# schlawg/fishnet

Measured on AMD Instinct MI355X. Metric: NNUE positions evaluated/sec (1–8 MI355X) + % HBM roofline, bit-exact, higher is better.
Workload: dtype int16

## Files before the change

### fishnet_amd/csrc/ft_sliced.hip

```cpp
#include <hip/hip_runtime.h>

#include <type_traits>

#include "sliced_common.h"

namespace fnnue {

namespace {

__global__ __launch_bounds__(1024) void plan_count_kernel(const fnnue_pos* __restrict__ pos, uint32_t n,
                                                         uint32_t* __restrict__ ctr, uint32_t* __restrict__ err) {
  __shared__ uint32_t h[kBins];
  for (int i = threadIdx.x; i < kBins; i += blockDim.x) h[i] = 0;
  __syncthreads();
  uint32_t bad = 0;
  for (uint32_t p = blockIdx.x * blockDim.x + threadIdx.x; p < n; p += gridDim.x * blockDim.x) {
    const LaneBoard b = lane_decode<false>(pos + p);
    if (!b.ok) {
      bad = 1;
      atomicAdd(&h[kItemBins + 8], 1u);
    } else {
      atomicAdd(&h[king_block(0, b.wk) * 33 + b.cnt], 1u);
      atomicAdd(&h[king_block(1, b.bk) * 33 + b.cnt], 1u);
      atomicAdd(&h[kItemBins + ((b.cnt - 1) >> 2)], 1u);
    }
  }
  if (__ballot(bad) && (threadIdx.x & 63) == 0) atomicOr(err, 1u);
  __syncthreads();
  for (int i = threadIdx.x; i < kBins; i += blockDim.x)
    if (h[i]) atomicAdd(&ctr[kCnt + i], h[i]);
}

__global__ __launch_bounds__(kScatterPositions) void plan_scatter_kernel(const fnnue_pos* __restrict__ pos, uint32_t n,
                                                           uint32_t* __restrict__ ctr, uint32_t* __restrict__ items,
                                                           uint16_t* __restrict__ flist, uint32_t* __restrict__ perm,
                                                           uint8_t* __restrict__ bucket_out,
                                                           int32_t* __restrict__ psqt_out) {
  __shared__ uint32_t lcnt[kBins];
  __shared__ uint32_t lbase[kBins];
  __shared__ uint32_t lists[kScatterPositions * kListStrideWords];
  for (int i = threadIdx.x; i < kBins; i += blockDim.x) lcnt[i] = 0;
  __syncthreads();
  const uint32_t p = blockIdx.x * kScatterPositions + threadIdx.x;
  const bool live = p < n;
  LaneBoard b;
  int kw = 0, kb = 0, kp = kItemBins + 8;
  uint32_t rw = 0, rb = 0, rp = 0;
  if (live) {
    b = lane_decode(pos + p);
    if (b.ok) {
      kw = king_block(0, b.wk) * 33 + b.cnt;
      kb = king_block(1, b.bk) * 33 + b.cnt;
      kp = kItemBins + ((b.cnt - 1) >> 2);
      rw = atomicAdd(&lcnt[kw], 1u);
      rb = atomicAdd(&lcnt[kb], 1u);
    }
    rp = atomicAdd(&lcnt[kp], 1u);
  }
  __syncthreads();
  for (int i = threadIdx.x; i < kBins; i += blockDim.x)
    lbase[i] = lcnt[i] ? atomicAdd(&ctr[kCur + i], lcnt[i]) : 0;
  __syncthreads();
  if (!live) return;
  const uint32_t slot = lbase[kp] + rp;
  perm[slot] = p;
  if (!b.ok) {
    bucket_out[slot] = 0xFF;
    psqt_out[p] = 0;
    return;
  }
  const int bucket = (b.cnt - 1) >> 2;
  const uint32_t iw = lbase[kw] + rw, ib = lbase[kb] + rb;
  uint32_t* mine = lists + threadIdx.x * kListStrideWords;
  write_rows(b, 0, b.wk, iw, (iw - ctr[kOff + king_block(0, b.wk) * 33]) & 1u, mine, flist);
  write_rows(b, 1, b.bk, ib, (ib - ctr[kOff + king_block(1, b.bk) * 33]) & 1u, mine, flist);
  items[iw] = ((uint32_t)b.cnt << 24) | ((uint32_t)bucket << 21) | (slot << 1) | (uint32_t)(b.stm != 0);
  items[ib] = ((uint32_t)b.cnt << 24) | ((uint32_t)bucket << 21) | (slot << 1) | (uint32_t)(b.stm != 1);
  bucket_out[slot] = (uint8_t)bucket;
}

template <int HD, bool kSwar, bool kPsqt, int kPStride, bool kClaim>
__device__ __forceinline__ uint32_t slice_pass(const PassFetch& f, uint2* __restrict__ lb, int lane, int it_in_wave,
                                               int s, int q, const char* base, u16x4 b_lo, u16x4 b_hi, int krow,
                                               const int32_t* ptile, __amdgpu_buffer_rsrc_t psqt_rsrc,
                                               __amdgpu_buffer_rsrc_t x_rsrc, uint32_t* next_pass) {
  constexpr int kLastItemLane = 48;
  const uint32_t rec = f.rec;
  const int maxn = (int)(__builtin_amdgcn_readlane(rec, kLastItemLane) >> 24);
  uint32_t claim = 0;
  if constexpr (kClaim) claim = claim_passes(next_pass, lane);
  lb[lane] = f.lst;
  uint32_t e[16];
  const uint4* my = reinterpret_cast<const uint4*>(lb) + 4 * it_in_wave;
#pragma unroll
  for (int m = 0; m < 4; ++m) {
    const uint4 v = my[m];
    e[4 * m] = v.x;
    e[4 * m + 1] = v.y;
    e[4 * m + 2] = v.z;
    e[4 * m + 3] = v.w;
  }
  u16x4 lo = b_lo, hi = b_hi;
  rows_sum<kSwar>(maxn - 1, e, base, lo, hi);
  const uint32_t xoff = (rec & kItemRowMask) * (HD / 2) + 32 * s + 4 * q;
  const uint32_t xv = kSwar ? transform4_swar(lo, hi) : transform4(lo, hi);
  __builtin_amdgcn_raw_buffer_store_b32(xv, x_rsrc, xoff, 0, 0);
  if constexpr (kPsqt) {
    const uint32_t li = (uint32_t)lane >> 3;
    const int src = (int)(((li & 4u) << 3) + ((0x10041400u >> (8u * (li & 3u))) & 0xFFu));
    const uint32_t reci = (uint32_t)__builtin_amdgcn_ds_bpermute(src << 2, (int)rec);
    const int bk = (int)((reci >> 21) & 7u);
    auto pw = [&](uint32_t en) { return (uint32_t)ptile[psqt_tile_word((int)(en >> 4), bk, kPStride)]; };
    uint32_t a2 = (lane & 7) == 0 ? (uint32_t)ptile[psqt_tile_word(krow, bk, kPStride)] : 0u;
    a2 += pw(f.lst.x & 0xFFFFu) + pw(f.lst.x >> 16) + pw(f.lst.y & 0xFFFFu) + pw(f.lst.y >> 16);
    a2 += (uint32_t)__builtin_amdgcn_mov_dpp((int)a2, 0xB1, 0xF, 0xF, false);
    a2 += (uint32_t)__builtin_amdgcn_mov_dpp((int)a2, 0x4E, 0xF, 0xF, false);
    a2 += (uint32_t)__builtin_amdgcn_mov_dpp((int)a2, 0x141, 0xF, 0xF, false);
    __builtin_amdgcn_raw_buffer_store_b32((int32_t)a2, psqt_rsrc,
                                          (lane & 7) == 0 ? (reci & kItemRowMask) * 4u : kDroppedOffset, 0, 0);
  }
  return claim;
}

#define FT_SLICES_LDS(G)                                                                                      \
  __shared__ uint4 img[G::kTileU4];                                                                           \
  __shared__ int32_t ptile[psqt_tile_words(G::kTileRows)];         \
  __shared__ uint2 lbuf[16][64];                                 \
  __shared__ uint32_t next_pass;

template <int HD, bool kSwar, class G>
__device__ __forceinline__ void ft_slices_body(uint4* img, int32_t* ptile, uint2 (*lbuf)[64], uint32_t* next_pass,
                                               const uint4* __restrict__ tiles,
                                               const int16_t* __restrict__ ftb, const uint32_t* __restrict__ ctr,
                                               const int4* __restrict__ units, const uint32_t* __restrict__ items,
                                               const uint16_t* __restrict__ flist, const int32_t* __restrict__ psqw,
                                               int32_t* __restrict__ psqt_part, uint8_t* __restrict__ x) {
  constexpr int S = HD / 64;
  constexpr int kTileU4 = G::kTileU4;
  const uint32_t w = blockIdx.x;
  const uint32_t j = w >> 3;
  const uint32_t unit = (j / S) * 8 + (w & 7);
  const int s = (int)(j % S);
  if (unit >= ctr[G::kNUnitsWord]) return;
  const int4 u = units[unit];
  const int lane = threadIdx.x & 63;
  const int wv = __builtin_amdgcn_readfirstlane(threadIdx.x >> 6);
  int it_in_wave, q;
  lane_item(lane, it_in_wave, q);
  constexpr int kTileLoads = (kTileU4 + 1023) / 1024;
  constexpr int kPStride = psqt_tile_stride(G::kTileRows);
  constexpr int kPtileU4 = psqt_fill_chunks(G::kTileRows), kPtileRealU4 = G::kRows * kPsqtBuckets / 4;
  static_assert(kPtileU4 <= 2048, "PSQT tile loads: two per thread");
  static_assert(kPStride % 32 == 4, "bucket b's rows start on bank 4 b");
  const uint4* src = tiles + ((size_t)u.x * S + s) * kTileU4;
  uint4 t[kTileLoads];
#pragma unroll
  for (int k = 0; k < kTileLoads; ++k)
    t[k] = src[min((int)threadIdx.x + 1024 * k, kTileU4 - 1)];
  uint4 pt[2];
  const uint4* psrc = reinterpret_cast<const uint4*>(psqw + (size_t)u.x * G::kRows * kPsqtBuckets);
  if (s == 0) {
#pragma unroll
    for (int k = 0; k < 2; ++k) pt[k] = psrc[min((int)threadIdx.x + 1024 * k, kPtileRealU4 - 1)];
  }
  u16x4 b_lo = *reinterpret_cast<const u16x4*>(ftb + 32 * s + 4 * q);
  u16x4 b_hi = *reinterpret_cast<const u16x4*>(ftb + HD / 2 + 32 * s + 4 * q);
  const int krow = G::king_row(u.x);
  const char* lbase = reinterpret_cast<const char*>(img) + G::kPlaneBytes * q;
  uint2* lb = lbuf[wv];
  const __amdgpu_buffer_rsrc_t psqt_rsrc = __builtin_amdgcn_make_buffer_rsrc(psqt_part, 0, kBufferRange, kBufferFlags);
  const __amdgpu_buffer_rsrc_t x_rsrc = __builtin_amdgcn_make_buffer_rsrc(x, 0, kBufferAll, kBufferFlags);
  const __amdgpu_buffer_rsrc_t items_rsrc =
      __builtin_amdgcn_make_buffer_rsrc(const_cast<uint32_t*>(items), 0, kBufferAll, kBufferFlags);
  const __amdgpu_buffer_rsrc_t flist_rsrc =
      __builtin_amdgcn_make_buffer_rsrc(const_cast<uint16_t*>(flist), 0, kBufferAll, kBufferFlags);
  const int last = u.z - 1;
  int base_a = u.y + wv * 8, base_b = base_a + 128;
  PassFetch fa = fetch_pass(items_rsrc, flist_rsrc, base_a, last, lane, it_in_wave);
  PassFetch fb = fetch_pass(items_rsrc, flist_rsrc, base_b, last, lane, it_in_wave);
#pragma unroll
  for (int k = 0; k < kTileLoads; ++k)
    if ((int)threadIdx.x + 1024 * k < kTileU4) {
      uint4 v = t[k];
      if constexpr (kSwar) v = swar_tile_words(v);
      img[threadIdx.x + 1024 * k] = v;
    }
  if (s == 0) {
#pragma unroll
    for (int k = 0; k < 2; ++k) {
      const int i = (int)threadIdx.x + 1024 * k;
      if (i < kPtileU4) {
        const uint4 v = i < kPtileRealU4 ? pt[k] : make_uint4(0, 0, 0, 0);
        const int r = psqt_fill_row(i);
        ptile[psqt_tile_word(r, psqt_fill_bucket(i, 0), kPStride)] = (int32_t)v.x;
        ptile[psqt_tile_word(r, psqt_fill_bucket(i, 1), kPStride)] = (int32_t)v.y;
        ptile[psqt_tile_word(r, psqt_fill_bucket(i, 2), kPStride)] = (int32_t)v.z;
        ptile[psqt_tile_word(r, psqt_fill_bucket(i, 3), kPStride)] = (int32_t)v.w;
      }
    }
  }
  if (threadIdx.x == 0) *next_pass = claim_start();
  __syncthreads();
  uint32_t claim = claim_passes(next_pass, lane);
  {
    const u32x4 kv = *reinterpret_cast<const u32x4*>(lbase + 16 * krow);
    if constexpr (kSwar) {
      b_lo = swar_words(b_lo);
      b_hi = swar_words_hi(b_hi);
    }
    accum_row<kSwar>(kv, b_lo, b_hi);
    if constexpr (kSwar) {
      b_lo = __builtin_bit_cast(u16x4, __builtin_bit_cast(u32x2, b_lo) + kSwarOffset);
      b_hi = __builtin_bit_cast(u16x4, __builtin_bit_cast(u32x2, b_hi) + kSwarOffset);
    }
  }
  auto run = [&](auto psqt) {
    constexpr bool kPsqt = decltype(psqt)::value;
    constexpr bool kClaimB = kClaimPasses == 1;
    while (base_a < u.z) {
      const PassFetch cur = fa;
      const int na = u.y + 8 * claimed_pass(claim);
      fa = fetch_pass(items_rsrc, flist_rsrc, na, last, lane, it_in_wave);
      claim = slice_pass<HD, kSwar, kPsqt, kPStride, true>(cur, lb, lane, it_in_wave, s, q, lbase, b_lo, b_hi, krow, ptile,
                                                           psqt_rsrc, x_rsrc, next_pass);
      base_a = na;
      if (base_b >= u.z) break;
      const PassFetch cur2 = fb;
      const int nb = kClaimPasses == 1 ? u.y + 8 * claimed_pass(claim) : na + 8;
      fb = fetch_pass(items_rsrc, flist_rsrc, nb, last, lane, it_in_wave);
      const uint32_t c2 = slice_pass<HD, kSwar, kPsqt, kPStride, kClaimB>(cur2, lb, lane, it_in_wave, s, q, lbase, b_lo,
                                                                          b_hi, krow, ptile, psqt_rsrc, x_rsrc, next_pass);
      if constexpr (kClaimB) claim = c2;
      base_b = nb;
    }
  };
  if (s == 0)
    run(std::true_type{});
  else
    run(std::false_type{});
}

template <int HD, bool kSwar, class G = ChessGeom>
__global__ __launch_bounds__(1024) void ft_slices_kernel(const uint4* __restrict__ tiles,
                                                         const int16_t* __restrict__ ftb,
                                                         const uint32_t* __restrict__ ctr,
                                                         const int4* __restrict__ units,
                                                         const uint32_t* __restrict__ items,
                                                         const uint16_t* __restrict__ flist,
                                                         const int32_t* __restrict__ psqw,
                                                         int32_t* __restrict__ psqt_part,
                                                         uint8_t* __restrict__ x) {
  FT_SLICES_LDS(G)
  ft_slices_body<HD, kSwar, G>(img, ptile, lbuf, &next_pass, tiles, ftb, ctr, units, items, flist, psqw, psqt_part, x);
}

template <int HD, class G = ChessGeom>
__global__ __launch_bounds__(1024) void ft_slices_mixed_kernel(const uint4* __restrict__ tiles,
                                                               const int16_t* __restrict__ ftb,
                                                               const uint32_t* __restrict__ ctr,
                                                               const int4* __restrict__ units,
                                                               const uint32_t* __restrict__ items,
                                                               const uint16_t* __restrict__ flist,
                                                               const int32_t* __restrict__ psqw,
                                                               int32_t* __restrict__ psqt_part,
                                                               uint8_t* __restrict__ x, uint64_t swar) {
  constexpr int S = HD / 64;
  FT_SLICES_LDS(G)
  const uint32_t s = (blockIdx.x >> 3) % S;
  if ((swar >> s) & 1)
    ft_slices_body<HD, true, G>(img, ptile, lbuf, &next_pass, tiles, ftb, ctr, units, items, flist, psqw, psqt_part, x);
  else
    ft_slices_body<HD, false, G>(img, ptile, lbuf, &next_pass, tiles, ftb, ctr, units, items, flist, psqw, psqt_part, x);
}

template <int HD>
hipError_t relayout_t(const NetPtrs& net, void* tiles, hipStream_t stream) {
  hipLaunchKernelGGL((relayout_kernel<HD>), dim3(2048), dim3(256), 0, stream, net.ft_w, (uint4*)tiles);
  return hipGetLastError();
}

template <int HD, class G = ChessGeom>
hipError_t ft_slices_t(const SlicedPlan& P, const NetPtrs& net, uint8_t* x, uint32_t max_units, hipStream_t stream) {
  constexpr int S = HD / 64;
  const uint32_t groups = (max_units + 7) / 8;
  const uint64_t all = (uint64_t(1) << S) - 1;
  if ((P.swar & all) == all)
    hipLaunchKernelGGL((ft_slices_kernel<HD, true, G>), dim3(groups * 8 * S), dim3(1024), 0, stream,
                       (const uint4*)P.tiles, net.ft_bias, P.ctr, (const int4*)P.units, P.items, P.flist, net.psqt_w,
                       P.psqt_part, x);
  else if ((P.swar & all) == 0)
    hipLaunchKernelGGL((ft_slices_kernel<HD, false, G>), dim3(groups * 8 * S), dim3(1024), 0, stream,
                       (const uint4*)P.tiles, net.ft_bias, P.ctr, (const int4*)P.units, P.items, P.flist, net.psqt_w,
                       P.psqt_part, x);
  else
    hipLaunchKernelGGL((ft_slices_mixed_kernel<HD, G>), dim3(groups * 8 * S), dim3(1024), 0, stream,
                       (const uint4*)P.tiles, net.ft_bias, P.ctr, (const int4*)P.units, P.items, P.flist, net.psqt_w,
                       P.psqt_part, x, P.swar);
  return hipGetLastError();
}

template <int HD, class G>
hipError_t relayout_g(const NetPtrs& net, void* tiles, hipStream_t stream) {
  hipLaunchKernelGGL((relayout_kernel<HD, G>), dim3(2048), dim3(256), 0, stream, net.ft_w, (uint4*)tiles);
  return hipGetLastError();
}

}

size_t sliced_tiles_bytes(uint32_t hd) { return tile_uint4_count(hd) * sizeof(uint4); }
size_t sliced_ctr_words() { return (3 * kBins + 16 + 3) & ~(size_t)3; }
uint32_t sliced_max_units(uint32_t chunk) { return slice_max_units(2 * chunk, 32); }

#define FNNUE_HD_DISPATCH(hd, CALL) \
  switch (hd) {                     \
    case 128: return CALL(128);     \
    case 256: return CALL(256);     \
    case 512: return CALL(512);     \
    case 1024: return CALL(1024);   \
    case 1536: return CALL(1536);   \
    case 2048: return CALL(2048);   \
    case 2560: return CALL(2560);   \
    case 3072: return CALL(3072);   \
    default: return hipErrorInvalidValue; \
  }

hipError_t launch_relayout_sliced(uint32_t hd, const NetPtrs& net, void* tiles, hipStream_t stream) {
#define CALL(H) relayout_t<H>(net, tiles, stream)
  FNNUE_HD_DISPATCH(hd, CALL)
#undef CALL
}

hipError_t launch_sliced_plan(const fnnue_pos* pos, uint32_t n, const SlicedPlan& P, int32_t* psqt, uint8_t* bucket,
                              uint32_t* err, hipStream_t stream) {
  if (n == 0) return hipSuccess;
  hipError_t e = hipMemsetAsync(P.ctr, 0, sliced_ctr_words() * sizeof(uint32_t), stream);
  if (e != hipSuccess) return e;
  uint32_t blocks = (n + 1023) / 1024;
  if (blocks > 256) blocks = 256;
  hipLaunchKernelGGL(plan_count_kernel, dim3(blocks), dim3(1024), 0, stream, pos, n, P.ctr, err);
  if ((e = hipGetLastError()) != hipSuccess) return e;
  hipLaunchKernelGGL(plan_scan_kernel_t<32>, dim3(1), dim3(1024), 0, stream, P.ctr, (int4*)P.units, kUnitWork);
  if ((e = hipGetLastError()) != hipSuccess) return e;
  hipLaunchKernelGGL(plan_scatter_kernel, dim3((n + kScatterPositions - 1) / kScatterPositions), dim3(kScatterPositions), 0, stream,
                     pos, n, P.ctr, P.items, P.flist, P.perm, bucket, psqt);
  return hipGetLastError();
}

hipError_t launch_sliced_ft(uint32_t hd, uint32_t n, const NetPtrs& net, const SlicedPlan& P, uint8_t* x,
                            hipStream_t stream) {
  if (n == 0) return hipSuccess;
  const uint32_t mu = sliced_max_units(n);
#define CALL(H) ft_slices_t<H>(P, net, x, mu, stream)
  FNNUE_HD_DISPATCH(hd, CALL)
#undef CALL
}

size_t variant_tiles_bytes(uint32_t hd, int variant) {
  const int planes = variant == kVariantCrazyhouse ? VariantGeom<kVBoardRows + kVHandRows>::kTileU4
                                                   : VariantGeom<kVBoardRows>::kTileU4;
  return (size_t)64 * (hd / 64) * planes * sizeof(uint4);
}

#define FNNUE_VHD_DISPATCH(hd, CALL)      \
  switch (hd) {                           \
    case 256: return CALL(256);           \
    case 512: return CALL(512);           \
    case 1024: return CALL(1024);         \
    default: return hipErrorInvalidValue; \
  }
#define FNNUE_VARIANT_DISPATCH(variant, CALLG)                                   \
  if (variant == kVariantCrazyhouse) {                                          \
    using G = VariantGeom<kVBoardRows + kVHandRows>;                            \
    FNNUE_VHD_DISPATCH(hd, CALLG)                                               \
  } else if (variant_board_only(variant)) {                                     \
    using G = VariantGeom<kVBoardRows>;                                         \
    FNNUE_VHD_DISPATCH(hd, CALLG)                                               \
  }                                                                             \
  return hipErrorInvalidValue;

hipError_t launch_relayout_variant(uint32_t hd, int variant, const NetPtrs& net, void* tiles, hipStream_t stream) {
#define CALLG(H) relayout_g<H, G>(net, tiles, stream)
  FNNUE_VARIANT_DISPATCH(variant, CALLG)
#undef CALLG
}

hipError_t launch_variant_ft(uint32_t hd, int variant, uint32_t n, const NetPtrs& net, const SlicedPlan& P, uint8_t* x,
                             hipStream_t stream) {
  if (n == 0) return hipSuccess;
  const uint32_t mu = variant_max_units(n);
#define CALLG(H) ft_slices_t<H, G>(P, net, x, mu, stream)
  FNNUE_VARIANT_DISPATCH(variant, CALLG)
#undef CALLG
}

hipError_t launch_ft_sliced(uint32_t hd, const fnnue_pos* pos, uint32_t n, const NetPtrs& net, const SlicedPlan& P,
                            uint8_t* x, int32_t* psqt, uint8_t* bucket, uint32_t* err, hipStream_t stream,
                            hipEvent_t mid) {
  hipError_t e = launch_sliced_plan(pos, n, P, psqt, bucket, err, stream);
  if (e == hipSuccess && mid) e = hipEventRecord(mid, stream);
  return e != hipSuccess ? e : launch_sliced_ft(hd, n, net, P, x, stream);
}

}
```

### fishnet_amd/csrc/sliced_common.h

```cpp
#pragma once
#include <hip/hip_runtime.h>

#include "device_common.h"
#include "kernels.h"
#include "net.h"
#include "psqt_tile.h"
#include "slice_units.h"

namespace fnnue {
namespace {

static_assert(kPsqtTileBuckets == kPsqtBuckets, "psqt_tile.h lays out the net's PSQT buckets");

constexpr int kRowsPerBlock = 704;
constexpr int kTileRows = kRowsPerBlock + 1;
constexpr int kNoRow = kRowsPerBlock;
constexpr int kPlaneBytes = 11296;
constexpr int kPlaneU4 = kPlaneBytes / 16;
constexpr int kPlaneU4_ = kPlaneU4;
constexpr int kTileU4 = 8 * kPlaneU4;
constexpr uint32_t kNoEntry = 16 * kNoRow;
__host__ __device__ constexpr int king_row(int kb) { return 640 + 8 * (7 - (kb >> 2)) + (7 - (kb & 3)); }
constexpr int kItemBins = 32 * 33;
constexpr int kPosBins = 9;
constexpr int kBins = kItemBins + kPosBins;
#ifndef PLAN_WG
#define PLAN_WG 1024
#endif
constexpr int kScatterPositions = PLAN_WG;

constexpr uint32_t kItemRowMask = 0x1FFFFF;

constexpr int kCnt = 0, kOff = kBins, kCur = 2 * kBins, kNUnits = 3 * kBins;

struct ChessGeom {
  static constexpr int kRows = kRowsPerBlock, kPlaneU4 = kPlaneU4_, kBlocks = 32, kNUnitsWord = kNUnits;
  static constexpr int kTileRows = kRows + 1, kPlaneBytes = 16 * kPlaneU4, kTileU4 = 8 * kPlaneU4;
  __host__ __device__ static constexpr int king_row(int kb) { return fnnue::king_row(kb); }
};
constexpr int kVItemBins = 64 * 33, kVBins = kVItemBins + kPosBins;
constexpr int kVCnt = 0, kVOff = kVBins, kVCur = 2 * kVBins, kVNUnits = 3 * kVBins;
template <int R>
struct VariantGeom {
  static_assert(R % 16 == 0, "plane stride must stay 32 mod 256");
  static constexpr int kRows = R, kPlaneU4 = R + 2, kBlocks = 64, kNUnitsWord = kVNUnits;
  static constexpr int kTileRows = kRows + 1, kPlaneBytes = 16 * kPlaneU4, kTileU4 = 8 * kPlaneU4;
  __host__ __device__ static constexpr int king_row(int kb) { return 640 + kb; }
};

__device__ __forceinline__ void lane_item(int lane, int& item, int& q) {
  const int l = lane & 31, hi = (lane >> 5) * 4;
  if (l < 4) { item = 0; q = l; }
  else if (l < 12) { item = 2; q = l - 4; }
  else if (l < 16) { item = 0; q = l - 8; }
  else if (l < 20) { item = 3; q = l - 16; }
  else if (l < 28) { item = 1; q = l - 20; }
  else { item = 3; q = l - 24; }
  item += hi;
}

struct LaneBoard {
  uint32_t w[8];
  uint64_t occ;
  int stm, wk, bk, cnt;
  int nwk, nbk;
  bool sane;
  bool ok;
};

__device__ __forceinline__ uint32_t zero_nibbles(uint32_t y) {
  return ~(((y & 0x77777777u) + 0x77777777u) | y) & 0x88888888u;
}

__device__ __forceinline__ uint32_t nibble_bits(uint32_t z) {
  uint32_t m = z >> 3;
  m = (m | (m >> 3)) & 0x03030303u;
  m = (m | (m >> 6)) & 0x000F000Fu;
  return (m | (m >> 12)) & 0xFFu;
}

template <bool kOcc = true>
__device__ __forceinline__ LaneBoard lane_decode(const fnnue_pos* p) {
  LaneBoard b;
  const uint32_t* pw = reinterpret_cast<const uint32_t*>(p);
#pragma unroll
  for (int i = 0; i < 8; ++i) b.w[i] = pw[i];
  b.stm = (int)(pw[8] & 0xFF);
  b.occ = 0;
  int nwk = 0, nbk = 0, cnt = 0;
  uint32_t bad = 0;
  b.wk = b.bk = 0;
#pragma unroll
  for (int i = 0; i < 8; ++i) {
    const uint32_t w = b.w[i];
    const uint32_t occb = ~zero_nibbles(w) & 0x88888888u;
    if constexpr (kOcc) b.occ |= (uint64_t)nibble_bits(occb) << (8 * i);
    cnt += __popc(occb);
    const uint32_t kw = zero_nibbles(w ^ 0x66666666u), kb = zero_nibbles(w ^ 0xEEEEEEEEu);
    nwk += __popc(kw);
    nbk += __popc(kb);
    if (kw) b.wk = 8 * i + (__builtin_ctz(kw) >> 2);
    if (kb) b.bk = 8 * i + (__builtin_ctz(kb) >> 2);
    bad |= (w & (w >> 1) & (w >> 2) & 0x11111111u) | zero_nibbles(w ^ 0x88888888u);
  }
  b.cnt = cnt;
  b.nwk = nwk;
  b.nbk = nbk;
  b.sane = !bad && b.cnt <= 32 && b.stm <= 1;
  b.ok = b.sane && nwk == 1 && nbk == 1;
  return b;
}

__device__ __forceinline__ int nibble_at(const uint32_t (&w)[8], int s) {
  const int i = s >> 3;
  const uint32_t a = (i & 1) ? w[1] : w[0], c = (i & 1) ? w[3] : w[2];
  const uint32_t e = (i & 1) ? w[5] : w[4], g = (i & 1) ? w[7] : w[6];
  const uint32_t lo = (i & 2) ? c : a, hi = (i & 2) ? g : e;
  return (int)((((i & 4) ? hi : lo) >> (4 * (s & 7))) & 15u);
}

__host__ __device__ constexpr uint32_t seg_len_bin(uint32_t L) {
  return L <= 16 ? L - 1 : L <= 144 ? 16 + (L - 17) / 8 : 32;
}
#ifndef SEG_UNIT_PLIES
#define SEG_UNIT_PLIES 20480
#endif
#ifndef SEG_UNIT_PLIES_SMALL
#define SEG_UNIT_PLIES_SMALL 8192
#endif
#ifndef SEG_ROOT_COST
#define SEG_ROOT_COST 4
#endif
constexpr uint32_t kSegUnitPlies = SEG_UNIT_PLIES;
constexpr uint32_t kSegUnitPliesSmall = SEG_UNIT_PLIES_SMALL;
__host__ __device__ constexpr uint32_t seg_unit_plies_for(uint32_t hd) {
  return hd <= 256 ? kSegUnitPliesSmall : kSegUnitPlies;
}
constexpr uint32_t kSegRootCost = SEG_ROOT_COST;
__host__ __device__ constexpr uint32_t seg_bin_longest(uint32_t bin) {
  return bin < 16 ? bin + 1 : bin < 32 ? 8 * bin - 104 : 160;
}
__host__ __device__ constexpr uint32_t seg_bin_weight(uint32_t bin) { return seg_bin_longest(bin) + kSegRootCost; }

template <int C>
__host__ __device__ constexpr uint32_t seg_count_class(uint32_t nfeat) {
  return C == 1 ? 0u : nfeat > 29 ? 3u : nfeat > 25 ? 2u : nfeat > 20 ? 1u : 0u;
}

template <int KB, int NB>
__host__ __device__ constexpr int plan_scan_lds_words() {
  return (KB * NB + kPosBins) + 16 + KB * NB + KB + 1 + 2 * KB;
}
template <int KB, int NB = 33>
__device__ __forceinline__ void plan_scan_body(uint32_t* __restrict__ ctr, int4* __restrict__ units,
                                               uint32_t unit_work, uint32_t seg_plies, uint32_t* __restrict__ nu_out,
                                               uint32_t* __restrict__ lds) {
  constexpr int kIB = KB * NB, kB = kIB + kPosBins, kO = kB, kC = 2 * kB, kNU = 3 * kB;
  auto len_bin = [](int i) { return (i % NB) / (NB / 33); };
  uint32_t* s = lds;
  uint32_t* part = lds + kB;
  const int t = threadIdx.x;
  constexpr int per = (kB + 1023) / 1024;
  uint32_t local[per];
  uint32_t sum = 0;
  for (int k = 0; k < per; ++k) {
    const int i = t * per + k;
    local[k] = (i < kIB) ? ctr[i] : 0;
    sum += local[k];
  }
  const int lane = t & 63, wv = t >> 6;
  uint32_t incl = sum;
#pragma unroll
  for (int o = 1; o < 64; o <<= 1) {
    const uint32_t v = __shfl_up(incl, o, 64);
    if (lane >= o) incl += v;
  }
  if (lane == 63) part[wv] = incl;
  __syncthreads();
  uint32_t run = incl - sum;
  for (int w = 0; w < wv; ++w) run += part[w];
  for (int k = 0; k < per; ++k) {
    const int i = t * per + k;
    if (i < kIB) s[i] = run;
    run += local[k];
  }
  if (t == 0) {
    uint32_t r = 0;
    for (int b = 0; b < kPosBins; ++b) {
      s[kIB + b] = r;
      r += ctr[kIB + b];
    }
  }
  __syncthreads();
  if (!nu_out)
    for (int i = t; i < kB; i += 1024) {
      ctr[kO + i] = s[i];
      ctr[kC + i] = s[i];
    }
  auto kb_end = [&](int kb) -> uint32_t { return kb == KB - 1 ? s[KB * NB - 1] + ctr[KB * NB - 1] : s[(kb + 1) * NB]; };
  if (unit_work == 0) {
    uint32_t* pb = lds + kB + 16;
    uint32_t* ubase = lds + kB + 16 + kIB;
    for (int k = 0; k < per; ++k) {
      const int i = t * per + k;
      if (i < kIB) pb[i] = local[k] * seg_bin_weight(len_bin(i));
    }
    __syncthreads();
    if (t < KB) {
      uint32_t run = 0;
      for (int b = 0; b < NB; ++b) {
        const uint32_t v = pb[t * NB + b];
        pb[t * NB + b] = run;
        run += v;
      }
      const uint32_t mine = (run + seg_plies - 1) / seg_plies;
      uint32_t incl = mine;
#pragma unroll
      for (int o = 1; o < KB; o <<= 1) {
        const uint32_t v = __shfl_up(incl, o, KB);
        if (t >= o) incl += v;
      }
      ubase[t] = incl - mine;
      if (t == KB - 1) {
        ubase[KB] = incl;
        if (nu_out) *nu_out = incl;
        else ctr[kNU] = incl;
      }
    }
    __syncthreads();
    for (int k = 0; k < per; ++k) {
      const int i = t * per + k;
      if (i >= kIB || local[k] == 0) continue;
      const int kb = i / NB;
      const uint32_t w = seg_bin_weight(len_bin(i)), p0 = pb[i], p1 = p0 + local[k] * w;
      for (uint32_t u = (p0 + seg_plies - 1) / seg_plies; u * seg_plies < p1; ++u)
        units[ubase[kb] + u] = make_int4(kb, (int)(s[i] + (u * seg_plies - p0 + w - 1) / w), 0, 0);
    }
    __syncthreads();
    for (uint32_t v = t; v < ubase[KB]; v += 1024) {
      const int kb = units[v].x;
      units[v].z = v + 1 < ubase[kb + 1] ? units[v + 1].y : (int)kb_end(kb);
    }
  } else {
    uint32_t* pb = lds + kB + 16;
    uint32_t* ubase = pb + kIB;
    uint32_t* bw = ubase + KB + 1;
    uint32_t* bm = bw + KB;
    int* uw = reinterpret_cast<int*>(units);
    for (int k = 0; k < per; ++k) {
      const int i = t * per + k;
      if (i < kIB) pb[i] = local[k] * slice_item_cost(len_bin(i));
    }
    __syncthreads();
    if (t < KB) {
      uint32_t w = 0;
      for (int b = 0; b < NB; ++b) {
        const uint32_t v = pb[t * NB + b];
        pb[t * NB + b] = w;
        w += v;
      }
      uint32_t work = w;
#pragma unroll
      for (int o = 1; o < KB; o <<= 1) work += __shfl_xor(work, o, KB);
      const uint32_t W = slice_budget(work, kb_end(KB - 1), unit_work);
      const uint32_t m = slice_block_units(w, W);
      const uint32_t key = m ? w / m : 0;
      uint32_t first = 0, nu = 0;
      for (int j = 0; j < KB; ++j) {
        const uint32_t kj = __shfl(key, j, KB), mj = __shfl(m, j, KB);
        nu += mj;
        if (kj > key || (kj == key && j < t)) first += mj;
      }
      ubase[t] = first;
      bw[t] = w;
      bm[t] = m;
      if (t == 0) {
        ubase[KB] = nu;
        if (nu_out) *nu_out = nu;
        else ctr[kNU] = nu;
      }
      if (m) {
        const uint32_t e0 = 4 * slice_table_slot(first, nu), e1 = 4 * slice_table_slot(first + m - 1, nu);
        uw[e0] = t;
        uw[e0 + 1] = (int)s[t * NB];
        uw[e0 + 3] = 0;
        uw[e1 + 2] = (int)kb_end(t);
      }
    }
    __syncthreads();
    constexpr int kLanes = 1024 / KB;
    const int kb = t / kLanes;
    const uint32_t w = bw[kb], m = bm[kb], first = ubase[kb], nu = ubase[KB], b0 = s[kb * NB];
    for (uint32_t u = 1 + t % kLanes; u < m; u += kLanes) {
      const uint32_t target = slice_cut_work(u, w, m);
      int b = -1;
#pragma unroll
      for (int k = 0; k < NB; ++k) b += pb[kb * NB + k] <= target ? 1 : 0;
      const int i = kb * NB + b;
      const int at = (int)(b0 + slice_cut_item(target, pb[i], s[i] - b0, slice_item_cost(len_bin(i))));
      const uint32_t e0 = 4 * slice_table_slot(first + u, nu), e1 = 4 * slice_table_slot(first + u - 1, nu);
      uw[e0] = kb;
      uw[e0 + 1] = at;
      uw[e0 + 3] = 0;
      uw[e1 + 2] = at;
    }
  }
}

template <int KB, int NB = 33>
__global__ __launch_bounds__(1024) __attribute__((unused)) void plan_scan_kernel_t(uint32_t* __restrict__ ctr,
                                                                                  int4* __restrict__ units,
                                                                                  uint32_t unit_work,
                                                                                  uint32_t seg_plies = 0,
                                                                                  uint32_t* __restrict__ nu_out = nullptr) {
  __shared__ uint32_t lds[plan_scan_lds_words<KB, NB>()];
  plan_scan_body<KB, NB>(ctr, units, unit_work, seg_plies, nu_out, lds);
}

constexpr int kListStrideWords = 17;

__host__ __device__ constexpr uint64_t plane_table(int persp) {
  uint64_t t = 0;
  for (int pc = 1; pc < 16; ++pc) {
    const int type = pc & 7;
    if (type < 1 || type > 6) continue;
    const int plane = type == 6 ? 10 : 2 * (type - 1) + ((pc >> 3) != persp);
    t |= (uint64_t)plane << (4 * pc);
  }
  return t;
}

__device__ __forceinline__ void write_rows(const LaneBoard& b, int persp, int ksq, uint32_t it, uint32_t pp,
                                               uint32_t* __restrict__ mine, uint16_t* __restrict__ flist) {
  const uint32_t mirror = (ksq & 7) < 4 ? 1u : 0u;
  const uint32_t flip = (persp ? 56u : 0u) ^ (mirror ? 7u : 0u);
  const uint64_t ptab = persp ? plane_table(1) : plane_table(0);
  constexpr uint64_t kEvenFiles = 0x5555555555555555ull;
  const uint32_t fpar = pp ^ mirror;
  const uint64_t occ = b.occ & ~(1ull << ksq);
  uint32_t kf = 0, ks = (uint32_t)__popcll(occ & (fpar ? ~kEvenFiles : kEvenFiles));
  typedef uint16_t u16_alias __attribute__((__may_alias__));
  typedef uint32_t u32_alias __attribute__((__may_alias__));
  u32_alias* M = reinterpret_cast<u32_alias*>(mine);
  u16_alias* L = reinterpret_cast<u16_alias*>(mine);
#pragma unroll
  for (int j = 0; j < 16; ++j) M[j] = kNoEntry | kNoEntry << 16;
  const uint32_t kw = (uint32_t)ksq >> 3, kbit = 1u << (4 * (ksq & 7));
#pragma unroll
  for (int i = 0; i < 8; ++i) {
    const uint32_t w = b.w[i];
    uint32_t nz = ((((w & 0x77777777u) + 0x77777777u) | w) >> 3) & 0x11111111u;
    nz &= kw == (uint32_t)i ? ~kbit : ~0u;
    const uint32_t c16 = ((8u * (uint32_t)i) ^ flip) << 4;
    while (nz) {
      const uint32_t bit = (uint32_t)__builtin_ctz(nz);
      nz &= nz - 1;
      const uint32_t plane = (uint32_t)(ptab >> (((w >> bit) & 15u) << 2)) & 15u;
      const uint32_t e = ((bit << 2) ^ c16) + (plane << 10);
      const bool f = ((bit >> 2) & 1u) == fpar;
      L[f ? kf : ks] = (uint16_t)e;
      kf += f ? 1u : 0u;
      ks += f ? 0u : 1u;
    }
  }
  uint4* dst = reinterpret_cast<uint4*>(flist + (size_t)it * 32);
#pragma unroll
  for (int q = 0; q < 4; ++q) dst[q] = make_uint4(M[4 * q], M[4 * q + 1], M[4 * q + 2], M[4 * q + 3]);
}

__host__ __device__ constexpr size_t tile_uint4_count(uint32_t hd) { return (size_t)32 * (hd / 64) * kTileU4; }

template <int HD, class G = ChessGeom>
__global__ __launch_bounds__(256) void relayout_kernel(const int16_t* __restrict__ ftw, uint4* __restrict__ tiles) {
  constexpr int S = HD / 64;
  constexpr size_t total = (size_t)G::kBlocks * S * G::kTileU4;
  for (size_t i = blockIdx.x * (size_t)blockDim.x + threadIdx.x; i < total; i += (size_t)gridDim.x * blockDim.x) {
    const int r = (int)(i % G::kPlaneU4);
    const size_t t = i / G::kPlaneU4;
    const int q = (int)(t & 7);
    const size_t ks = t >> 3;
    const int s = (int)(ks % S), kb = (int)(ks / S);
    uint4 v = make_uint4(0, 0, 0, 0);
    if (r < G::kRows) {
      const int16_t* row = ftw + (size_t)(kb * G::kRows + r) * HD;
      const uint2 lo = *reinterpret_cast<const uint2*>(row + 32 * s + 4 * q);
      const uint2 hi = *reinterpret_cast<const uint2*>(row + HD / 2 + 32 * s + 4 * q);
      v = make_uint4(lo.x, lo.y, hi.x, hi.y);
    }
    tiles[i] = v;
  }
}

constexpr int kBufferRange = 0x7FFFFFFF;
constexpr int kBufferFlags = 0x00020000;
constexpr int kBufferAll = -1;
constexpr uint32_t kDroppedOffset = 0x80000000u;

typedef unsigned short u16x4 __attribute__((ext_vector_type(4)));
typedef unsigned int u32x4 __attribute__((ext_vector_type(4)));
typedef unsigned int u32x2 __attribute__((ext_vector_type(2)));
typedef short s16x4 __attribute__((ext_vector_type(4)));

__device__ __forceinline__ uint32_t transform4(u16x4 lo, u16x4 hi) {
  const s16x4 zero = (s16x4)0, top = (s16x4)127;
  const s16x4 a = __builtin_elementwise_min(__builtin_elementwise_max((s16x4)lo, zero), top);
  const s16x4 b = __builtin_elementwise_min(__builtin_elementwise_max((s16x4)hi, zero), top);
  const u16x4 pr = ((u16x4)a * (u16x4)b) << (u16x4)1;
  const u32x2 w = __builtin_bit_cast(u32x2, pr);
  return __builtin_amdgcn_perm(w.y, w.x, 0x07050301u);
}

struct PassFetch {
  uint32_t rec;
  uint2 lst;
};
__device__ __forceinline__ PassFetch fetch_pass(__amdgpu_buffer_rsrc_t items, __amdgpu_buffer_rsrc_t flist,
                                                int pass_base, int last, int lane, int it_in_wave) {
  PassFetch f;
  f.rec = __builtin_amdgcn_raw_buffer_load_b32(items, (uint32_t)min(pass_base + it_in_wave, last) * 4u, 0, 0);
  const uint32_t li = (uint32_t)min(pass_base + (lane >> 3), last);
  const u32x2 l = __builtin_amdgcn_raw_buffer_load_b64(flist, li * 64u + 8u * (uint32_t)(lane & 7), 0, 0);
  f.lst = make_uint2(l.x, l.y);
  return f;
}

#ifndef FT_CLAIM
#define FT_CLAIM 2
#endif
constexpr int kClaimPasses = FT_CLAIM;
static_assert(kClaimPasses == 1 || kClaimPasses == 2, "FT_CLAIM: 1 or 2 passes per claim");
constexpr uint32_t claim_start() { return 32 / kClaimPasses; }
__device__ __forceinline__ uint32_t claim_passes(uint32_t* next_claim, int lane) {
  uint32_t c = 0;
  if (lane == 0) c = __builtin_amdgcn_atomic_inc32(next_claim, 0xFFFFFFFFu, __ATOMIC_RELAXED, "workgroup");
  return c;
}
__device__ __forceinline__ int claimed_pass(uint32_t claim) {
  return kClaimPasses * __builtin_amdgcn_readfirstlane((int)claim);
}

__device__ __forceinline__ const u32x4* row_addr(const char* base, uint32_t word, int t) {
  const uint32_t entry = (t & 1) ? (word >> 16) : (word & 0xFFFFu);
  return static_cast<const u32x4*>(__builtin_assume_aligned(base + entry, 16));
}

#ifndef FT_DEPTH
#define FT_DEPTH 2
#endif
constexpr int kRowDepth = 4 * FT_DEPTH;

__device__ __forceinline__ uint32_t swar_word(uint32_t packed) { return packed - ((packed & 0x8000u) << 1); }
__device__ __forceinline__ u16x4 swar_words(u16x4 v) {
  const u32x2 w = __builtin_bit_cast(u32x2, v);
  return __builtin_bit_cast(u16x4, u32x2{swar_word(w.x), swar_word(w.y)});
}

constexpr uint32_t kSwarOffset = 0x80008000u;
__device__ __forceinline__ uint32_t swar_word_hi(uint32_t packed) {
  return swar_word((packed << 1) & 0xFFFEFFFEu);
}
__device__ __forceinline__ u16x4 swar_words_hi(u16x4 v) {
  const u32x2 w = __builtin_bit_cast(u32x2, v);
  return __builtin_bit_cast(u16x4, u32x2{swar_word_hi(w.x), swar_word_hi(w.y)});
}
__device__ __forceinline__ uint4 swar_tile_words(uint4 v) {
  return make_uint4(swar_word(v.x), swar_word(v.y), swar_word_hi(v.z), swar_word_hi(v.w));
}
__device__ __forceinline__ uint32_t transform4_swar(u16x4 lo, u16x4 hi) {
  const u16x4 off = (u16x4)0x8000, top = (u16x4)127, top2 = (u16x4)254;
  const u16x4 a = __builtin_elementwise_min(__builtin_elementwise_sub_sat(lo, off), top);
  const u16x4 b2 = __builtin_elementwise_min(__builtin_elementwise_sub_sat(hi, off), top2);
  const u32x2 w = __builtin_bit_cast(u32x2, a * b2);
  return __builtin_amdgcn_perm(w.y, w.x, 0x07050301u);
}

template <bool kSwar = false>
__device__ __forceinline__ void accum_row(const u32x4& v, u16x4& lo, u16x4& hi) {
  const u32x2 a = __builtin_shufflevector(v, v, 0, 1);
  const u32x2 b = __builtin_shufflevector(v, v, 2, 3);
  if constexpr (kSwar) {
    lo = __builtin_bit_cast(u16x4, __builtin_bit_cast(u32x2, lo) + a);
    hi = __builtin_bit_cast(u16x4, __builtin_bit_cast(u32x2, hi) + b);
  } else {
    lo += __builtin_bit_cast(u16x4, a);
    hi += __builtin_bit_cast(u16x4, b);
  }
}

template <int NR, int R = 0>
__device__ __forceinline__ void rows1_head(const uint32_t (&e)[16], const char* base, u32x4 (&v)[kRowDepth]) {
  if constexpr (R < NR && R < kRowDepth) {
    v[R] = *row_addr(base, e[R >> 1], R & 1);
    rows1_head<NR, R + 1>(e, base, v);
  }
}

template <int NR, bool kSwar, int R = 0>
__device__ __forceinline__ void rows1_step(const uint32_t (&e)[16], const char* base, u32x4 (&v)[kRowDepth],
                                           u16x4& lo, u16x4& hi) {
  if constexpr (R < NR) {
    accum_row<kSwar>(v[R % kRowDepth], lo, hi);
    if constexpr (R + kRowDepth < NR) v[R % kRowDepth] = *row_addr(base, e[(R + kRowDepth) >> 1], (R + kRowDepth) & 1);
    rows1_step<NR, kSwar, R + 1>(e, base, v, lo, hi);
  }
}

template <int NR, bool kSwar>
__device__ __forceinline__ void rows_exact(const uint32_t (&e)[16], const char* base, u16x4& lo, u16x4& hi) {
  u32x4 v[kRowDepth];
  rows1_head<NR>(e, base, v);
  rows1_step<NR, kSwar>(e, base, v, lo, hi);
}

template <bool kSwar = false>
__device__ __forceinline__ void rows_sum(int nrows, const uint32_t (&e)[16], const char* base, u16x4& lo, u16x4& hi) {
  switch (nrows) {
#define FNNUE_ROWS_CASE(k) \
  case k: rows_exact<k, kSwar>(e, base, lo, hi); break;
    FNNUE_ROWS_CASE(1) FNNUE_ROWS_CASE(2) FNNUE_ROWS_CASE(3) FNNUE_ROWS_CASE(4) FNNUE_ROWS_CASE(5)
    FNNUE_ROWS_CASE(6) FNNUE_ROWS_CASE(7) FNNUE_ROWS_CASE(8) FNNUE_ROWS_CASE(9) FNNUE_ROWS_CASE(10)
    FNNUE_ROWS_CASE(11) FNNUE_ROWS_CASE(12) FNNUE_ROWS_CASE(13) FNNUE_ROWS_CASE(14) FNNUE_ROWS_CASE(15)
    FNNUE_ROWS_CASE(16) FNNUE_ROWS_CASE(17) FNNUE_ROWS_CASE(18) FNNUE_ROWS_CASE(19) FNNUE_ROWS_CASE(20)
    FNNUE_ROWS_CASE(21) FNNUE_ROWS_CASE(22) FNNUE_ROWS_CASE(23) FNNUE_ROWS_CASE(24) FNNUE_ROWS_CASE(25)
    FNNUE_ROWS_CASE(26) FNNUE_ROWS_CASE(27) FNNUE_ROWS_CASE(28) FNNUE_ROWS_CASE(29) FNNUE_ROWS_CASE(30)
    FNNUE_ROWS_CASE(31) FNNUE_ROWS_CASE(32)
#undef FNNUE_ROWS_CASE
    default: break;
  }
}

}
}
```

Measured before the change: 800.0 million.

## Walk board once for both perspectives and overlap it with global atomics

The scatter kernel now decodes each board's piece list once in a shared walk_board pass and derives both perspectives' feature lists from it by XOR transforms, instead of running write_rows twice. The global atomicAdd for bin bases and the ctr offset loads are issued before the board walk and their results are written to LDS afterwards, so atomic latency overlaps the walk. Occupancy is also pinned to 8 waves per EU. The cost is more register pressure from holding the walked list and per-lane bases across the barrier, plus a second list-building code path guarded by static_asserts that tie it to the existing tables.

```diff
diff --git a/fishnet_amd/csrc/ft_sliced.hip b/fishnet_amd/csrc/ft_sliced.hip
--- a/fishnet_amd/csrc/ft_sliced.hip
+++ b/fishnet_amd/csrc/ft_sliced.hip
@@ -31,7 +31,8 @@
     if (h[i]) atomicAdd(&ctr[kCnt + i], h[i]);
 }
 
-__global__ __launch_bounds__(kScatterPositions) void plan_scatter_kernel(const fnnue_pos* __restrict__ pos, uint32_t n,
+__global__ __launch_bounds__(kScatterPositions) __attribute__((amdgpu_waves_per_eu(8, 8)))
+void plan_scatter_kernel(const fnnue_pos* __restrict__ pos, uint32_t n,
                                                            uint32_t* __restrict__ ctr, uint32_t* __restrict__ items,
                                                            uint16_t* __restrict__ flist, uint32_t* __restrict__ perm,
                                                            uint8_t* __restrict__ bucket_out,
@@ -46,9 +47,11 @@
   LaneBoard b;
   int kw = 0, kb = 0, kp = kItemBins + 8;
   uint32_t rw = 0, rb = 0, rp = 0;
+  bool ok = false;
   if (live) {
     b = lane_decode(pos + p);
-    if (b.ok) {
+    ok = b.ok;
+    if (ok) {
       kw = king_block(0, b.wk) * 33 + b.cnt;
       kb = king_block(1, b.bk) * 33 + b.cnt;
       kp = kItemBins + ((b.cnt - 1) >> 2);
@@ -58,22 +61,39 @@
     rp = atomicAdd(&lcnt[kp], 1u);
   }
   __syncthreads();
-  for (int i = threadIdx.x; i < kBins; i += blockDim.x)
-    lbase[i] = lcnt[i] ? atomicAdd(&ctr[kCur + i], lcnt[i]) : 0;
+  constexpr int kBinsPerLane = (kBins + kScatterPositions - 1) / kScatterPositions;
+  uint32_t base[kBinsPerLane];
+#pragma unroll
+  for (int k = 0; k < kBinsPerLane; ++k) {
+    const int i = threadIdx.x + k * kScatterPositions;
+    const uint32_t c = i < kBins ? lcnt[i] : 0;
+    base[k] = c ? atomicAdd(&ctr[kCur + i], c) : 0;
+  }
+  uint32_t* mine = lists + threadIdx.x * kListStrideWords;
+  ListWalk walk{};
+  uint32_t firstw = 0, firstb = 0;
+  if (ok) {
+    firstw = ctr[kOff + king_block(0, b.wk) * 33];
+    firstb = ctr[kOff + king_block(1, b.bk) * 33];
+    walk = walk_board(b.w, b.occ, b.wk, b.bk, mine);
+  }
+#pragma unroll
+  for (int k = 0; k < kBinsPerLane; ++k) {
+    const int i = threadIdx.x + k * kScatterPositions;
+    if (i < kBins) lbase[i] = base[k];
+  }
   __syncthreads();
   if (!live) return;
   const uint32_t slot = lbase[kp] + rp;
   perm[slot] = p;
-  if (!b.ok) {
+  if (!ok) {
     bucket_out[slot] = 0xFF;
     psqt_out[p] = 0;
     return;
   }
   const int bucket = (b.cnt - 1) >> 2;
   const uint32_t iw = lbase[kw] + rw, ib = lbase[kb] + rb;
-  uint32_t* mine = lists + threadIdx.x * kListStrideWords;
-  write_rows(b, 0, b.wk, iw, (iw - ctr[kOff + king_block(0, b.wk) * 33]) & 1u, mine, flist);
-  write_rows(b, 1, b.bk, ib, (ib - ctr[kOff + king_block(1, b.bk) * 33]) & 1u, mine, flist);
+  emit_list_pair(walk, b.wk, b.bk, iw, (iw - firstw) & 1u, ib, (ib - firstb) & 1u, mine, flist);
   items[iw] = ((uint32_t)b.cnt << 24) | ((uint32_t)bucket << 21) | (slot << 1) | (uint32_t)(b.stm != 0);
   items[ib] = ((uint32_t)b.cnt << 24) | ((uint32_t)bucket << 21) | (slot << 1) | (uint32_t)(b.stm != 1);
   bucket_out[slot] = (uint8_t)bucket;
diff --git a/fishnet_amd/csrc/plan_lists.h b/fishnet_amd/csrc/plan_lists.h
--- /dev/null
+++ b/fishnet_amd/csrc/plan_lists.h
@@ -0,0 +1,115 @@
+#pragma once
+#include <stdint.h>
+
+#ifdef __HIPCC__
+#define FNNUE_HD __host__ __device__
+#define FNNUE_HD_INLINE __host__ __device__ __forceinline__
+#define FNNUE_UNROLL _Pragma("unroll")
+#else
+#define FNNUE_HD
+#define FNNUE_HD_INLINE inline
+#define FNNUE_UNROLL
+#endif
+
+namespace fnnue {
+
+constexpr uint32_t kListRows = 704;
+constexpr uint32_t kListNoEntry = 16 * kListRows;
+constexpr int kListWalked = 30;
+
+FNNUE_HD constexpr uint64_t white_plane_table() {
+  uint64_t t = 0;
+  for (int pc = 1; pc < 16; ++pc) {
+    const int type = pc & 7;
+    if (type < 1 || type > 5) continue;
+    t |= (uint64_t)(2 * (type - 1) + (pc >> 3)) << (4 * pc);
+  }
+  return t;
+}
+
+struct alignas(16) ListQuad {
+  uint32_t x, y, z, w;
+} __attribute__((__may_alias__));
+
+struct ListWalk {
+  uint32_t v[kListWalked / 2];
+  uint64_t pcs;
+  uint32_t n;
+};
+
+FNNUE_HD_INLINE ListWalk walk_board(const uint32_t (&w)[8], uint64_t occ, int wk, int bk, uint32_t* __restrict__ mine) {
+  typedef uint16_t u16_alias __attribute__((__may_alias__));
+  typedef uint32_t u32_alias __attribute__((__may_alias__));
+  u32_alias* M = reinterpret_cast<u32_alias*>(mine);
+  u16_alias* L = reinterpret_cast<u16_alias*>(mine);
+  constexpr uint64_t ptab = white_plane_table();
+  ListWalk r;
+  const uint64_t pcs = occ & ~(1ull << wk) & ~(1ull << bk);
+  r.pcs = pcs;
+  r.n = (uint32_t)__builtin_popcount((uint32_t)pcs) + (uint32_t)__builtin_popcount((uint32_t)(pcs >> 32));
+  uint32_t at = 0;
+FNNUE_UNROLL
+  for (int h = 0; h < 2; ++h) {
+    uint32_t m = (uint32_t)(pcs >> (32 * h));
+    const uint32_t wa = w[4 * h], wb = w[4 * h + 1], wc = w[4 * h + 2], wd = w[4 * h + 3];
+    while (m) {
+      const uint32_t j = (uint32_t)__builtin_ctz(m);
+      m &= m - 1;
+      const uint32_t lo = (j & 8u) ? wb : wa, hi = (j & 8u) ? wd : wc;
+      const uint32_t nib = (((j & 16u) ? hi : lo) >> ((j & 7u) << 2)) & 15u;
+      const uint32_t plane = (uint32_t)(ptab >> (nib << 2)) & 15u;
+      L[at++] = (uint16_t)((32u * h + j) | plane << 6);
+    }
+  }
+FNNUE_UNROLL
+  for (int j = 0; j < kListWalked / 2; ++j) r.v[j] = M[j];
+  return r;
+}
+
+FNNUE_HD_INLINE void emit_list_pair(const ListWalk& r, int wk, int bk, uint32_t itw, uint32_t ppw, uint32_t itb,
+                                    uint32_t ppb, uint32_t* __restrict__ mine, uint16_t* __restrict__ flist) {
+  typedef uint16_t u16_alias __attribute__((__may_alias__));
+  typedef uint32_t u32_alias __attribute__((__may_alias__));
+  u32_alias* M = reinterpret_cast<u32_alias*>(mine);
+  u16_alias* L = reinterpret_cast<u16_alias*>(mine);
+  constexpr uint64_t kEvenFiles = 0x5555555555555555ull;
+  const uint64_t pcs = r.pcs;
+  const uint32_t n = r.n;
+  const uint32_t m0 = (wk & 7) < 4 ? 7u : 0u, m1 = (bk & 7) < 4 ? 7u : 0u;
+  auto emit = [&](uint32_t fx, uint32_t king_t, int king_sq, uint32_t mirror, uint32_t pp, uint32_t it) {
+FNNUE_UNROLL
+    for (int j = 0; j < 16; ++j) M[j] = kListNoEntry | kListNoEntry << 16;
+    const uint64_t first_files = (pp ^ (mirror & 1u)) ? ~kEvenFiles : kEvenFiles;
+    const uint64_t firsts = (pcs | 1ull << king_sq) & first_files;
+    u16_alias* pf = L;
+    u16_alias* ps = L + (uint32_t)__builtin_popcount((uint32_t)firsts) + (uint32_t)__builtin_popcount((uint32_t)(firsts >> 32));
+    auto put = [&](uint32_t e, uint32_t s) {
+      *(s ? ps : pf) = (uint16_t)e;
+      ps += s;
+      pf += 1u - s;
+    };
+    put(king_t << 4, (king_t ^ pp) & 1u);
+    const uint32_t fx2 = fx | fx << 16, pp2 = pp | pp << 16;
+FNNUE_UNROLL
+    for (int k = 0; k < kListWalked; ++k) {
+      if ((uint32_t)k >= n) break;
+      const uint32_t t2 = r.v[k >> 1] ^ fx2;
+      const uint32_t e2 = t2 << 4, s2 = (t2 ^ pp2) & 0x00010001u;
+      put((k & 1) ? e2 >> 16 : e2, (k & 1) ? s2 >> 16 : s2 & 1u);
+    }
+    ListQuad* dst = static_cast<ListQuad*>(__builtin_assume_aligned(flist + (size_t)it * 32, 16));
+FNNUE_UNROLL
+    for (int q = 0; q < 4; ++q) dst[q] = ListQuad{M[4 * q], M[4 * q + 1], M[4 * q + 2], M[4 * q + 3]};
+  };
+  const uint32_t fx0 = m0, fx1 = 56u ^ m1 ^ 64u;
+  emit(fx0, ((uint32_t)bk | 10u << 6) ^ fx0, bk, m0, ppw, itw);
+  emit(fx1, ((uint32_t)wk | 10u << 6) ^ fx1 ^ 64u, wk, m1, ppb, itb);
+}
+
+FNNUE_HD_INLINE void build_list_pair(const uint32_t (&w)[8], uint64_t occ, int wk, int bk, uint32_t itw, uint32_t ppw,
+                                     uint32_t itb, uint32_t ppb, uint32_t* __restrict__ mine,
+                                     uint16_t* __restrict__ flist) {
+  emit_list_pair(walk_board(w, occ, wk, bk, mine), wk, bk, itw, ppw, itb, ppb, mine, flist);
+}
+
+}
diff --git a/fishnet_amd/csrc/sliced_common.h b/fishnet_amd/csrc/sliced_common.h
--- a/fishnet_amd/csrc/sliced_common.h
+++ b/fishnet_amd/csrc/sliced_common.h
@@ -4,6 +4,7 @@
 #include "device_common.h"
 #include "kernels.h"
 #include "net.h"
+#include "plan_lists.h"
 #include "psqt_tile.h"
 #include "slice_units.h"
 
@@ -329,6 +330,8 @@
   }
   return t;
 }
+static_assert(kListNoEntry == kNoEntry && kListRows == kRowsPerBlock, "plan_lists.h: the zero row");
+static_assert((plane_table(0) & 0xF0FFFFFFF0FFFFFFull) == white_plane_table(), "plan_lists.h: white's planes, kings aside");
 
 __device__ __forceinline__ void write_rows(const LaneBoard& b, int persp, int ksq, uint32_t it, uint32_t pp,
                                                uint32_t* __restrict__ mine, uint16_t* __restrict__ flist) {
```

Result: faster. 808.3 million (median of 6 runs) (+1.0%).
